# leavesnight/VIEO_SLAM

Hardware: AMD Instinct MI355X
Metric: frontend+localBA frames/sec on EuRoC MH05 stereo-VIO; ATE vs ref (higher is better)
Workload: dtype u8 (extract/match) + f64 (pose optimisation)

## Files before the change

vieo_slam_amd/csrc/matching.hip:

```cpp
#include <climits>

#include "orb_internal.h"
#include "wave_ops.h"

namespace vieo {

static const int TH_HIGH = 100, TH_LOW = 50;

__device__ __forceinline__ int hamming32(const uint4 a0, const uint4 a1, const uint8_t* b) {
  const uint4 b0 = ((const uint4*)b)[0], b1 = ((const uint4*)b)[1];
  return __popc(a0.x ^ b0.x) + __popc(a0.y ^ b0.y) + __popc(a0.z ^ b0.z) + __popc(a0.w ^ b0.w) +
         __popc(a1.x ^ b1.x) + __popc(a1.y ^ b1.y) + __popc(a1.z ^ b1.z) + __popc(a1.w ^ b1.w);
}

__device__ __forceinline__ bool lex_less(int d0, int i0, int d1, int i1) {
  return d0 < d1 || (d0 == d1 && i0 < i1);
}

struct Knn2Job {
  const uint8_t* q;
  const uint8_t* t;
  int nq, nt;
  int out_off;
};

struct Knn2Src {
  const Knn2Job* jobs;
  const uint8_t* desc;
  const int32_t* counts;
  int cap, n_cams, n_pairs;
  signed char pi[6], pj[6];
};

__global__ void __launch_bounds__(256)
k_knn2(Knn2Src S, int32_t* __restrict__ idx, int32_t* __restrict__ dist) {
  __shared__ uint4 s_t[256 * 2];
  __shared__ unsigned s_m[3][64][2];
  Knn2Job J;
  if (S.jobs)
    J = S.jobs[blockIdx.y];
  else {
    const int f = blockIdx.z, p = blockIdx.y, ci = S.pi[p], cj = S.pj[p];
    const int32_t* c = S.counts + (size_t)f * S.n_cams * 2;
    const int ni = c[2 * ci], mi = c[2 * ci + 1], nj = c[2 * cj], mj = c[2 * cj + 1];
    const bool skip = mi >= ni || mj >= nj;
    J.q = S.desc + (((size_t)f * S.n_cams + ci) * S.cap + mi) * 32;
    J.t = S.desc + (((size_t)f * S.n_cams + cj) * S.cap + mj) * 32;
    J.nq = skip ? 0 : min(ni, S.cap) - mi, J.nt = skip ? 0 : min(nj, S.cap) - mj;
    J.out_off = ((int)f * S.n_pairs + p) * S.cap;
  }
  const int lane = threadIdx.x & 63, wave = __builtin_amdgcn_readfirstlane((int)(threadIdx.x >> 6));
  const int q0 = blockIdx.x * 64;
  if (q0 >= J.nq) return;
  const int qi = q0 + lane;
  uint4 a0 = {0, 0, 0, 0}, a1 = a0;
  if (qi < J.nq) a0 = ((const uint4*)(J.q + (size_t)qi * 32))[0], a1 = ((const uint4*)(J.q + (size_t)qi * 32))[1];
  unsigned k0 = 0xFFFFFFFFu, k1 = 0xFFFFFFFFu;
  const uint4* T = (const uint4*)J.t;
  for (int t0 = 0; t0 < J.nt; t0 += 256) {
    __syncthreads();
    const int rows = min(256, J.nt - t0);
    for (int e = threadIdx.x; e < rows * 2; e += 256) s_t[e] = T[(size_t)t0 * 2 + e];
    __syncthreads();
    const int r1 = min(rows, wave * 64 + 64);
    for (int r = wave * 64; r < r1; r++) {
      const uint4 b0 = s_t[2 * r], b1 = s_t[2 * r + 1];
      const unsigned d = __popc(a0.x ^ b0.x) + __popc(a0.y ^ b0.y) + __popc(a0.z ^ b0.z) + __popc(a0.w ^ b0.w) +
                         __popc(a1.x ^ b1.x) + __popc(a1.y ^ b1.y) + __popc(a1.z ^ b1.z) + __popc(a1.w ^ b1.w);
      const unsigned key = (d << 16) | (unsigned)(t0 + r);
      k1 = min(max(key, k0), k1);
      k0 = min(k0, key);
    }
  }
  if (wave > 0) s_m[wave - 1][lane][0] = k0, s_m[wave - 1][lane][1] = k1;
  __syncthreads();
  if (wave == 0 && qi < J.nq) {
#pragma unroll
    for (int w = 0; w < 3; w++) {
      const unsigned b0 = s_m[w][lane][0], b1 = s_m[w][lane][1];
      const unsigned lo = min(k0, b0), hi = max(k0, b0);
      k1 = min(hi, min(k1, b1));
      k0 = lo;
    }
    int32_t* oi = idx + ((size_t)J.out_off + qi) * 2;
    int32_t* od = dist + ((size_t)J.out_off + qi) * 2;
    oi[0] = k0 == 0xFFFFFFFFu ? -1 : (int)(k0 & 0xFFFF), od[0] = k0 == 0xFFFFFFFFu ? INT_MAX : (int)(k0 >> 16);
    oi[1] = k1 == 0xFFFFFFFFu ? -1 : (int)(k1 & 0xFFFF), od[1] = k1 == 0xFFFFFFFFu ? INT_MAX : (int)(k1 >> 16);
  }
}

typedef int knn_v16i __attribute__((ext_vector_type(16)));
typedef int knn_v4i __attribute__((ext_vector_type(4)));

__device__ __forceinline__ unsigned knn_spread4(unsigned nib) { return (nib * 0x00204081u) & 0x01010101u; }
__device__ __forceinline__ knn_v4i knn_spread16(unsigned h) {
  knn_v4i r;
  r[0] = (int)knn_spread4(h & 15u), r[1] = (int)knn_spread4((h >> 4) & 15u);
  r[2] = (int)knn_spread4((h >> 8) & 15u), r[3] = (int)knn_spread4((h >> 12) & 15u);
  return r;
}

#ifndef VIEO_KNN2_TILE_ROWS
#define VIEO_KNN2_TILE_ROWS 32
#endif
__global__ void __launch_bounds__(256)
k_knn2_mfma(Knn2Src S, int32_t* __restrict__ idx, int32_t* __restrict__ dist) {
  constexpr int TR = VIEO_KNN2_TILE_ROWS, NSUB = TR / 32, CH = TR * 16;
  __shared__ knn_v4i s_a[2][CH];
  __shared__ __attribute__((aligned(16))) unsigned s_L[2][TR];
  Knn2Job J;
  if (S.jobs)
    J = S.jobs[blockIdx.y];
  else {
    const int f = blockIdx.z, p = blockIdx.y, ci = S.pi[p], cj = S.pj[p];
    const int32_t* c = S.counts + (size_t)f * S.n_cams * 2;
    const int ni = c[2 * ci], mi = c[2 * ci + 1], nj = c[2 * cj], mj = c[2 * cj + 1];
    const bool skip = mi >= ni || mj >= nj;
    J.q = S.desc + (((size_t)f * S.n_cams + ci) * S.cap + mi) * 32;
    J.t = S.desc + (((size_t)f * S.n_cams + cj) * S.cap + mj) * 32;
    J.nq = skip ? 0 : min(ni, S.cap) - mi, J.nt = skip ? 0 : min(nj, S.cap) - mj;
    J.out_off = ((int)f * S.n_pairs + p) * S.cap;
  }
  if ((int)blockIdx.x * 256 >= J.nq) return;
  const int tid = threadIdx.x, lane = tid & 63, wave = tid >> 6;
  const int j = lane & 31, g = lane >> 5;
  const int q0 = blockIdx.x * 256 + wave * 64;
  knn_v4i B[2][8];
  unsigned pb[2];
#pragma unroll
  for (int s = 0; s < 2; s++) {
    const int qi = q0 + 32 * s + j;
    uint4 h = {0, 0, 0, 0};
    if (qi < J.nq) h = ((const uint4*)(J.q + (size_t)qi * 32))[g];
    const unsigned half = __popc(h.x) + __popc(h.y) + __popc(h.z) + __popc(h.w);
    pb[s] = half + (unsigned)__shfl_xor((int)half, 32);
    const unsigned w[4] = {h.x, h.y, h.z, h.w};
#pragma unroll
    for (int m = 0; m < 8; m++) B[s][m] = knn_spread16((w[m >> 1] >> (16 * (m & 1))) & 0xFFFFu);
  }
  unsigned k0[2] = {0xFFFFFFFFu, 0xFFFFFFFFu}, k1[2] = {0xFFFFFFFFu, 0xFFFFFFFFu};
  const int n_tiles = (J.nt + TR - 1) / TR;
  constexpr int NU = CH / 256;
  unsigned h16[NU];
  uint4 ra = {0, 0, 0, 0}, rb = ra;
  auto fetch = [&](int T) {
#pragma unroll
    for (int u = 0; u < NU; u++) {
      const int cc = tid + 256 * u, sub = cc >> 9, m = (cc >> 6) & 7, gg = (cc >> 5) & 1, row = T * TR + sub * 32 + (cc & 31);
      h16[u] = row < J.nt ? (unsigned)*(const unsigned short*)(J.t + (size_t)row * 32 + 16 * gg + 2 * m) : 0u;
    }
    if (tid < TR) {
      const int row = T * TR + tid;
      ra = rb = make_uint4(0, 0, 0, 0);
      if (row < J.nt) ra = ((const uint4*)(J.t + (size_t)row * 32))[0], rb = ((const uint4*)(J.t + (size_t)row * 32))[1];
    }
  };
  auto stage = [&](int T, int b) {
#pragma unroll
    for (int u = 0; u < NU; u++) s_a[b][tid + 256 * u] = knn_spread16(h16[u]);
    if (tid < TR) {
      const int row = T * TR + tid;
      const unsigned pa = __popc(ra.x) + __popc(ra.y) + __popc(ra.z) + __popc(ra.w) + __popc(rb.x) + __popc(rb.y) + __popc(rb.z) + __popc(rb.w);
      s_L[b][tid] = row < J.nt ? ((pa + 512u) << 16) | (unsigned)row : 0xFFFFFFFFu;
    }
  };
  fetch(0);
  stage(0, 0);
  __syncthreads();
  for (int T = 0; T < n_tiles; T++) {
    const int b = T & 1;
    if (T + 1 < n_tiles) fetch(T + 1);
#pragma unroll
    for (int sub = 0; sub < NSUB; sub++) {
      knn_v16i acc0 = {0, 0, 0, 0, 0, 0, 0, 0, 0, 0, 0, 0, 0, 0, 0, 0}, acc1 = acc0;
#pragma unroll
      for (int m = 0; m < 8; m++) {
        const knn_v4i a = s_a[b][((sub * 8 + m) * 2 + g) * 32 + j];
        acc0 = __builtin_amdgcn_mfma_i32_32x32x32_i8(a, B[0][m], acc0, 0, 0, 0);
        acc1 = __builtin_amdgcn_mfma_i32_32x32x32_i8(a, B[1][m], acc1, 0, 0, 0);
      }
#pragma unroll
      for (int q4 = 0; q4 < 4; q4++) {
        const uint4 Lw = *(const uint4*)&s_L[b][sub * 32 + 8 * q4 + 4 * g];
        const unsigned L[4] = {Lw.x, Lw.y, Lw.z, Lw.w};
#pragma unroll
        for (int e = 0; e < 4; e++) {
          const unsigned ka = L[e] - ((unsigned)acc0[4 * q4 + e] << 17), kb = L[e] - ((unsigned)acc1[4 * q4 + e] << 17);
          k1[0] = min(max(ka, k0[0]), k1[0]), k0[0] = min(k0[0], ka);
          k1[1] = min(max(kb, k0[1]), k1[1]), k0[1] = min(k0[1], kb);
        }
      }
    }
    if (T + 1 < n_tiles) stage(T + 1, b ^ 1);
    __syncthreads();
  }
#pragma unroll
  for (int s = 0; s < 2; s++) {
    const unsigned o0 = (unsigned)__shfl_xor((int)k0[s], 32), o1 = (unsigned)__shfl_xor((int)k1[s], 32);
    const unsigned lo = min(k0[s], o0), hi = max(k0[s], o0);
    const unsigned second = min(hi, min(k1[s], o1));
    const int qi = q0 + 32 * s + j;
    if (g == 0 && qi < J.nq) {
      int32_t* oi = idx + ((size_t)J.out_off + qi) * 2;
      int32_t* od = dist + ((size_t)J.out_off + qi) * 2;
      oi[0] = lo == 0xFFFFFFFFu ? -1 : (int)(lo & 0xFFFF), od[0] = lo == 0xFFFFFFFFu ? INT_MAX : (int)(lo >> 16) - 512 + (int)pb[s];
      oi[1] = second == 0xFFFFFFFFu ? -1 : (int)(second & 0xFFFF);
      od[1] = second == 0xFFFFFFFFu ? INT_MAX : (int)(second >> 16) - 512 + (int)pb[s];
    }
  }
}

static bool knn2_mfma() {
  static const bool on = [] {
    const char* e = getenv("VIEO_KNN2_MFMA");
    return !e || atoi(e) != 0;
  }();
  return on;
}
static void knn2_launch(const Knn2Src& S, int max_nq, int ny, int nz, int32_t* d_idx, int32_t* d_dist, hipStream_t st) {
  if (knn2_mfma())
    hipLaunchKernelGGL(k_knn2_mfma, dim3((max_nq + 255) / 256, ny, nz), dim3(256), 0, st, S, d_idx, d_dist);
  else
    hipLaunchKernelGGL(k_knn2, dim3((max_nq + 63) / 64, ny, nz), dim3(256), 0, st, S, d_idx, d_dist);
}

int knn2_rig_launch(const uint8_t* d_desc, const int32_t* d_counts, int cap, int n_cams, int n_frames, int32_t* d_idx,
                    int32_t* d_dist, hipStream_t st) {
  Knn2Src S;
  memset(&S, 0, sizeof(S));
  S.desc = d_desc, S.counts = d_counts, S.cap = cap, S.n_cams = n_cams;
  int p = 0;
  for (int i = 0; i < n_cams - 1; i++)
    for (int j = i + 1; j < n_cams; j++, p++) S.pi[p] = (signed char)i, S.pj[p] = (signed char)j;
  S.n_pairs = p;
  if (p == 0 || n_frames <= 0) return VIEO_OK;
  knn2_launch(S, cap, p, n_frames, d_idx, d_dist, st);
  VIEO_HIP_CHECK(hipGetLastError());
  return VIEO_OK;
}

struct StereoArgs {
  OrbParams P;
  ImgSet IL, IR;
  int l_first, l_step, r_first, r_step;
  const vieo_keypoint *kpL, *kpR;
  const uint8_t *descL, *descR;
  const int *cntL, *cntR;
  int capL, capR;
  float baseline, bf;
  float* uright;
  float* depth;
  int* sad;
  int* row_start;
  int2* row_list;
  int H, list_cap;
};

__device__ __forceinline__ int wave_sum_i(int v) { return wave_sum_i32(v); }

template <int NT>
__global__ void __launch_bounds__(NT) k_stereo_rows(StereoArgs A) {
  extern __shared__ int s_rows[];
  __shared__ int s_part[16];
  const int f = blockIdx.x, tid = threadIdx.x, H = A.H;
  int* cnt = s_rows;
  int* cur = s_rows + H + 1;
  const int imR = A.r_first + f * A.r_step;
  const int Nr = min(A.cntR[2 * imR], A.capR);
  const vieo_keypoint* KR = A.kpR + (size_t)imR * A.capR;
  for (int y = tid; y <= H; y += NT) cnt[y] = 0;
  __syncthreads();
  for (int j = tid; j < Nr; j += NT) {
    const float y = KR[j].y, r = 2.0f * A.P.lv[KR[j].octave].scale;
    const int maxr = min((int)ceilf(y + r), H - 1), minr = max((int)floorf(y - r), 0);
    for (int yi = minr; yi <= maxr; yi++) atomicAdd(&cnt[yi], 1);
  }
  __syncthreads();
  const int per = (H + NT - 1) / NT, y0 = min(H, tid * per), y1 = min(H, y0 + per);
  int sum = 0;
  for (int y = y0; y < y1; y++) sum += cnt[y];
  int inc = sum;
  for (int o = 1; o < 64; o <<= 1) {
    const int t = __shfl_up(inc, o);
    if ((tid & 63) >= o) inc += t;
  }
  if ((tid & 63) == 63) s_part[tid >> 6] = inc;
  __syncthreads();
  int acc = inc - sum;
  for (int w = 0; w < (tid >> 6); w++) acc += s_part[w];
  int* rs = A.row_start + (size_t)f * (H + 1);
  for (int y = y0; y < y1; y++) {
    const int v = cnt[y];
    rs[y] = acc, cur[y] = acc;
    acc += v;
  }
  if (tid == NT - 1) rs[H] = acc;
  __syncthreads();
  int2* list = A.row_list + (size_t)f * A.list_cap;
  for (int j = tid; j < Nr; j += NT) {
    const vieo_keypoint kj = KR[j];
    const float y = kj.y, r = 2.0f * A.P.lv[kj.octave].scale;
    const int maxr = min((int)ceilf(y + r), H - 1), minr = max((int)floorf(y - r), 0);
    for (int yi = minr; yi <= maxr; yi++) {
      const int pos = atomicAdd(&cur[yi], 1);
      if (pos < A.list_cap) list[pos] = make_int2(j | (kj.octave << 20), __float_as_int(kj.x));
    }
  }
}

__device__ __forceinline__ unsigned row_min_u32(unsigned v) {
  v = min(v, (unsigned)VIEO_DPP(v, v, VIEO_DPP_QUAD_XOR1, 0xF));
  v = min(v, (unsigned)VIEO_DPP(v, v, VIEO_DPP_QUAD_XOR2, 0xF));
  v = min(v, (unsigned)VIEO_DPP(v, v, VIEO_DPP_ROW_HALF_MIRROR, 0xF));
  v = min(v, (unsigned)VIEO_DPP(v, v, VIEO_DPP_ROW_MIRROR, 0xF));
  return v;
}
__device__ __forceinline__ int row_sum_i32(int v) {
  v += VIEO_DPP(0, v, VIEO_DPP_QUAD_XOR1, 0xF);
  v += VIEO_DPP(0, v, VIEO_DPP_QUAD_XOR2, 0xF);
  v += VIEO_DPP(0, v, VIEO_DPP_ROW_HALF_MIRROR, 0xF);
  v += VIEO_DPP(0, v, VIEO_DPP_ROW_MIRROR, 0xF);
  return v;
}

__global__ void __launch_bounds__(256) k_stereo_rect(StereoArgs A) {
  const int f = blockIdx.y, lane = threadIdx.x & 63, g = lane >> 4, gl = lane & 15;
  const int wave = __builtin_amdgcn_readfirstlane((int)(threadIdx.x >> 6));
  const int iL = (blockIdx.x * 4 + wave) * 4 + g;
  const int imL = A.l_first + f * A.l_step, imR = A.r_first + f * A.r_step;
  const int N = min(A.cntL[2 * imL], A.capL);
  bool alive = iL < N;
  const int iLc = alive ? iL : 0;
  float* o_ur = A.uright + (size_t)f * A.capL + iLc;
  float* o_dp = A.depth + (size_t)f * A.capL + iLc;
  int* o_sad = A.sad + (size_t)f * A.capL + iLc;
  if (alive && gl == 0) *o_ur = -1.0f, *o_dp = -1.0f, *o_sad = -1;
  if (!__any(alive)) return;
  const vieo_keypoint kL = A.kpL[(size_t)imL * A.capL + iLc];
  const int levelL = kL.octave;
  const float vL = kL.y, uL = kL.x;
  const int rowL = (int)vL;
  const float minD = 0.f, maxD = A.bf / A.baseline;
  const float minU = uL - maxD, maxU = uL - minD;
  alive = alive && !(maxU < 0) && rowL >= 0 && rowL < A.H;
  const int rowc = min(max(rowL, 0), A.H - 1);
  const uint8_t* dL = A.descL + ((size_t)imL * A.capL + iLc) * 32;
  const uint4 a0 = ((const uint4*)dL)[0], a1 = ((const uint4*)dL)[1];
  const uint8_t* DR = A.descR + (size_t)imR * A.capR * 32;
  int bestDist = TH_HIGH, bestIdx = INT_MAX;
  float bestX = 0.f;
  const int* rs = A.row_start + (size_t)f * (A.H + 1);
  const int2* list = A.row_list + (size_t)f * A.list_cap;
  const int c0 = rs[rowc], c1 = alive ? min(rs[rowc + 1], A.list_cap) : c0;
  for (int cb = c0; __any(cb < c1); cb += 32) {
    int2 e[2];
    bool in[2];
#pragma unroll
    for (int u = 0; u < 2; u++) {
      const int c = cb + gl + 16 * u;
      in[u] = c < c1;
      e[u] = in[u] ? list[c] : make_int2(0, 0);
    }
    int dd[2];
#pragma unroll
    for (int u = 0; u < 2; u++) {
      const int j = e[u].x & 0xFFFFF, octR = e[u].x >> 20;
      const float xR = __int_as_float(e[u].y);
      in[u] = in[u] && !(octR < levelL - 1 || octR > levelL + 1) && (xR >= minU && xR <= maxU);
      dd[u] = in[u] ? hamming32(a0, a1, DR + (size_t)j * 32) : TH_HIGH;
    }
#pragma unroll
    for (int u = 0; u < 2; u++) {
      const int j = e[u].x & 0xFFFFF;
      if (in[u] && dd[u] < TH_HIGH && lex_less(dd[u], j, bestDist, bestIdx))
        bestDist = dd[u], bestIdx = j, bestX = __int_as_float(e[u].y);
    }
  }
  const int myIdx = bestIdx;
  {
    const unsigned m = row_min_u32(bestIdx == INT_MAX ? 0xFFFFFFFFu : ((unsigned)bestDist << 20) | (unsigned)bestIdx);
    bestIdx = m == 0xFFFFFFFFu ? INT_MAX : (int)(m & 0xFFFFF);
    bestDist = m == 0xFFFFFFFFu ? INT_MAX : (int)(m >> 20);
  }
  alive = alive && bestIdx != INT_MAX && bestDist < (TH_HIGH + TH_LOW) / 2;
  const unsigned long long own = __ballot(alive && myIdx == bestIdx);
  const unsigned own_g = (unsigned)((own >> (16 * g)) & 0xFFFFull);
  const int src_lane = g * 16 + (own_g ? __builtin_ffs((int)own_g) - 1 : 0);
  const float uR0 = __int_as_float(__builtin_amdgcn_ds_bpermute(src_lane * 4, __float_as_int(bestX)));
  const float sF = 1.0f / A.P.lv[levelL].scale;
  const float scaleduL = roundf(kL.x * sF), scaledvL = roundf(kL.y * sF);
  const float scaleduR0 = roundf(uR0 * sF);
  const int w = 5, L = 5;
  const float iniu = scaleduR0 + L - w, endu = scaleduR0 + L + w + 1;
  const int lvw = A.P.lv[levelL].w, lvh = A.P.lv[levelL].h;
  alive = alive && !(iniu < 0 || endu >= (float)lvw);
  if (!__any(alive)) return;
  int pitchL, pitchR;
  const uint8_t* PL = plane_ptr(A.P, A.IL, imL, levelL, &pitchL);
  const uint8_t* PR = plane_ptr(A.P, A.IR, imR, levelL, &pitchR);
  const int r0 = (int)(scaledvL - w), cL0 = (int)(scaleduL - w), cR0 = (int)(scaleduR0 - w);
  auto clampy = [&](int yy) { return min(max(yy, 0), lvh - 1); };
  auto clampx = [&](int xx) { return min(max(xx, 0), lvw - 1); };
  const int cvL = alive ? (int)PL[(size_t)(r0 + w) * pitchL + cL0 + w] : 0;
  int py[8], px[8], il[8];
#pragma unroll
  for (int k = 0; k < 8; k++) {
    const int p = gl + 16 * k;
    py[k] = p / 11, px[k] = p - py[k] * 11;
    il[k] = (alive && p < 121) ? (int)PL[(size_t)clampy(r0 + py[k]) * pitchL + clampx(cL0 + px[k])] - cvL : 0;
  }
  __shared__ uint8_t s_strip[16][11 * 21 + 25];
  uint8_t* strip = s_strip[wave * 4 + g];
  {
    unsigned v[15];
#pragma unroll
    for (int k = 0; k < 15; k++) {
      const int p = gl + 16 * k, row = p / 21, col = p - row * 21;
      v[k] = (alive && p < 231) ? PR[(size_t)clampy(r0 + row) * pitchR + clampx(cR0 - L + col)] : 0;
    }
#pragma unroll
    for (int k = 0; k < 15; k++)
      if (gl + 16 * k < 231) strip[gl + 16 * k] = (uint8_t)v[k];
  }
  __builtin_amdgcn_fence(__ATOMIC_RELEASE, "wavefront");
  __builtin_amdgcn_wave_barrier();
  __builtin_amdgcn_fence(__ATOMIC_ACQUIRE, "wavefront");
  int bestS = INT_MAX, bestInc = 0, sads[11];
#pragma unroll
  for (int inc = -L; inc <= L; inc++) {
    const int cvR = strip[w * 21 + inc + L + w];
    int acc = 0;
#pragma unroll
    for (int k = 0; k < 8; k++) {
      if (gl + 16 * k < 121) {
        const int ir = (int)strip[py[k] * 21 + inc + L + px[k]] - cvR;
        acc += abs(il[k] - ir);
      }
    }
    acc = row_sum_i32(acc);
    sads[inc + L] = acc;
    if (acc < bestS) bestS = acc, bestInc = inc;
  }
  if (!alive || bestInc == -L || bestInc == L) return;
  float dist1 = 0, dist2 = 0, dist3 = 0;
#pragma unroll
  for (int k = 1; k < 10; k++)
    if (k == bestInc + L) dist1 = (float)sads[k - 1], dist2 = (float)sads[k], dist3 = (float)sads[k + 1];
  const float deltaR = (dist1 - dist3) / (2.0f * (dist1 + dist3 - 2.0f * dist2));
  if (deltaR < -1 || deltaR > 1) return;
  float bestuR = A.P.lv[levelL].scale * ((float)scaleduR0 + (float)bestInc + deltaR);
  float disparity = uL - bestuR;
  if (disparity >= minD && disparity < maxD) {
    if (disparity <= 0) {
      disparity = 0.01f;
      bestuR = (float)((double)uL - 0.01);
    }
    if (gl == 0) {
      *o_dp = A.bf / disparity;
      *o_ur = bestuR;
      *o_sad = bestS;
    }
  }
}

__global__ void __launch_bounds__(256) k_stereo_median(StereoArgs A) {
  __shared__ int s_part[2][4];
  const int f = blockIdx.x, tid = threadIdx.x, lane = tid & 63, wave = tid >> 6;
  const int imL = A.l_first + f * A.l_step;
  const int N = min(A.cntL[2 * imL], A.capL);
  int* sad = A.sad + (size_t)f * A.capL;
  constexpr int kR = 8;
  int v[kR];
#pragma unroll
  for (int r = 0; r < kR; r++) {
    const int i = tid + 256 * r;
    v[r] = i < N ? sad[i] : -1;
  }
  const bool spill = N > 256 * kR;
  auto block_count = [&](int bound, int slot) -> int {
    int c = 0;
#pragma unroll
    for (int r = 0; r < kR; r++) c += (v[r] >= 0 && v[r] <= bound);
    if (spill)
      for (int i = tid + 256 * kR; i < N; i += 256) {
        const int s = sad[i];
        c += (s >= 0 && s <= bound);
      }
    c = wave_sum_i32(c);
    if (lane == 0) s_part[slot][wave] = c;
    __syncthreads();
    return s_part[slot][0] + s_part[slot][1] + s_part[slot][2] + s_part[slot][3];
  };
  const int n = block_count((1 << 30), 0);
  if (n == 0) return;
  const int k = n / 2;
  int lo = 0, hi = (1 << 17) - 1;
  int slot = 1;
  while (lo < hi) {
    const int mid = (lo + hi) >> 1;
    const int cnt = block_count(mid, slot);
    slot ^= 1;
    if (cnt >= k + 1)
      hi = mid;
    else
      lo = mid + 1;
  }
  const float median = (float)lo;
  const float thDist = 1.5f * 1.4f * median;
  for (int i = tid; i < N; i += 256) {
    const int s = sad[i];
    if (s >= 0 && !((float)s < thDist)) {
      A.uright[(size_t)f * A.capL + i] = -1;
      A.depth[(size_t)f * A.capL + i] = -1;
    }
  }
}

static thread_local DevBuf g_row_start, g_row_list;

static int launch_stereo(StereoArgs A, int n_frames, hipStream_t st) {
  int rc;
  float smax = 1.f;
  for (int l = 0; l < A.P.nlevels; l++) smax = std::max(smax, A.P.lv[l].scale);
  A.H = A.P.lv[0].h;
  if (A.capR >= (1 << 20)) {
    set_error("ComputeStereoMatches: more than 2^20 keys per image");
    return VIEO_E_CAPACITY;
  }
  A.list_cap = A.capR * (2 * (int)ceilf(2.0f * smax) + 3);
  if ((rc = g_row_start.ensure((size_t)n_frames * (A.H + 1) * 4)) != VIEO_OK) return rc;
  if ((rc = g_row_list.ensure((size_t)n_frames * A.list_cap * 8)) != VIEO_OK) return rc;
  A.row_start = g_row_start.as<int>(), A.row_list = g_row_list.as<int2>();
  if (n_frames <= 16)
    hipLaunchKernelGGL(k_stereo_rows<1024>, dim3(n_frames), dim3(1024), (size_t)(2 * A.H + 1) * 4, st, A);
  else
    hipLaunchKernelGGL(k_stereo_rows<256>, dim3(n_frames), dim3(256), (size_t)(2 * A.H + 1) * 4, st, A);
  hipLaunchKernelGGL(k_stereo_rect, dim3((A.capL + 15) / 16, n_frames), dim3(256), 0, st, A);
  hipLaunchKernelGGL(k_stereo_median, dim3(n_frames), dim3(256), 0, st, A);
  VIEO_HIP_CHECK(hipGetLastError());
  return VIEO_OK;
}

static int same_geometry(const vieo_orb* a, const vieo_orb* b) {
  if (a->w != b->w || a->h != b->h || a->nlevels != b->nlevels || a->w == 0) return 0;
  for (int l = 0; l < a->nlevels; l++)
    if (a->P.lv[l].w != b->P.lv[l].w || a->P.lv[l].h != b->P.lv[l].h ||
        a->P.lv[l].scale != b->P.lv[l].scale)
      return 0;
  return 1;
}

struct MatchScratch {
  DevBuf kpL, kpR, dL, dR, cL, cR, ur, dp, sad, jobs, idx, dist;
};
static thread_local MatchScratch g_ms;

}

using namespace vieo;

extern "C" {

int vieo_stereo_match_rectified_batch_device(vieo_orb* e, int n_frames,
                                             const vieo_keypoint* d_keypoints,
                                             const uint8_t* d_descriptors, const int32_t* d_counts,
                                             int capacity, float baseline, float bf,
                                             float* d_uright, float* d_depth) {
  if (!e || n_frames <= 0 || 2 * n_frames > e->last_B || !d_keypoints || !d_descriptors ||
      !d_counts || !d_uright || !d_depth || !(baseline > 0) || !(bf > 0)) {
    set_error("vieo_stereo_match_rectified_batch_device: invalid arguments (the extractor's last "
              "batch must hold 2*n_frames images, left/right interleaved)");
    return VIEO_E_INVALID;
  }
  int rc;
  static thread_local DevBuf sad;
  if ((rc = sad.ensure((size_t)n_frames * capacity * 4)) != VIEO_OK) return rc;
  StereoArgs A;
  A.P = e->P;
  A.IL = A.IR = e->last_imgs;
  A.l_first = 0, A.l_step = 2, A.r_first = 1, A.r_step = 2;
  A.kpL = A.kpR = d_keypoints;
  A.descL = A.descR = d_descriptors;
  A.cntL = A.cntR = d_counts;
  A.capL = A.capR = capacity;
  A.baseline = baseline;
  A.bf = bf;
  A.uright = d_uright;
  A.depth = d_depth;
  A.sad = sad.as<int>();
  return launch_stereo(A, n_frames, e->stream);
}

int vieo_stereo_match_rectified(vieo_orb* left, vieo_orb* right, const vieo_keypoint* h_kpL,
                                const uint8_t* h_descL, int nL, const vieo_keypoint* h_kpR,
                                const uint8_t* h_descR, int nR, float baseline, float bf,
                                float* h_uright, float* h_depth) {
  if (!left || !right || nL < 0 || nR < 0 || !h_uright || !h_depth || !(baseline > 0) || !(bf > 0))
    return VIEO_E_INVALID;
  if (left->last_B < 1 || right->last_B < 1 || !same_geometry(left, right)) {
    set_error("vieo_stereo_match_rectified: both extractors must have processed equally sized "
              "images (their pyramids are read in place)");
    return VIEO_E_INVALID;
  }
  if (nL == 0) return VIEO_OK;
  int rc;
  MatchScratch& S = g_ms;
  const int capL = nL, capR = std::max(nR, 1);
#define ENS(b, n) \
  if ((rc = (b).ensure(n)) != VIEO_OK) return rc
  ENS(S.kpL, (size_t)capL * sizeof(vieo_keypoint));
  ENS(S.kpR, (size_t)capR * sizeof(vieo_keypoint));
  ENS(S.dL, (size_t)capL * 32);
  ENS(S.dR, (size_t)capR * 32);
  ENS(S.cL, 8);
  ENS(S.cR, 8);
  ENS(S.ur, (size_t)capL * 4);
  ENS(S.dp, (size_t)capL * 4);
  ENS(S.sad, (size_t)capL * 4);
#undef ENS
  hipStream_t st = left->stream;
  VIEO_HIP_CHECK(hipStreamSynchronize(right->stream));
  const int cl[2] = {nL, 0}, cr[2] = {nR, 0};
  VIEO_HIP_CHECK(hipMemcpyAsync(S.kpL.p, h_kpL, (size_t)nL * sizeof(vieo_keypoint), hipMemcpyHostToDevice, st));
  VIEO_HIP_CHECK(hipMemcpyAsync(S.dL.p, h_descL, (size_t)nL * 32, hipMemcpyHostToDevice, st));
  if (nR > 0) {
    VIEO_HIP_CHECK(hipMemcpyAsync(S.kpR.p, h_kpR, (size_t)nR * sizeof(vieo_keypoint), hipMemcpyHostToDevice, st));
    VIEO_HIP_CHECK(hipMemcpyAsync(S.dR.p, h_descR, (size_t)nR * 32, hipMemcpyHostToDevice, st));
  }
  VIEO_HIP_CHECK(hipMemcpyAsync(S.cL.p, cl, 8, hipMemcpyHostToDevice, st));
  VIEO_HIP_CHECK(hipMemcpyAsync(S.cR.p, cr, 8, hipMemcpyHostToDevice, st));
  StereoArgs A;
  A.P = left->P;
  A.IL = left->last_imgs;
  A.IR = right->last_imgs;
  A.l_first = 0, A.l_step = 0, A.r_first = 0, A.r_step = 0;
  A.kpL = S.kpL.as<vieo_keypoint>(), A.kpR = S.kpR.as<vieo_keypoint>();
  A.descL = S.dL.as<uint8_t>(), A.descR = S.dR.as<uint8_t>();
  A.cntL = S.cL.as<int>(), A.cntR = S.cR.as<int>();
  A.capL = capL, A.capR = capR;
  A.baseline = baseline, A.bf = bf;
  A.uright = S.ur.as<float>(), A.depth = S.dp.as<float>(), A.sad = S.sad.as<int>();
  if ((rc = launch_stereo(A, 1, st)) != VIEO_OK) return rc;
  VIEO_HIP_CHECK(hipMemcpyAsync(h_uright, S.ur.p, (size_t)nL * 4, hipMemcpyDeviceToHost, st));
  VIEO_HIP_CHECK(hipMemcpyAsync(h_depth, S.dp.p, (size_t)nL * 4, hipMemcpyDeviceToHost, st));
  VIEO_HIP_CHECK(hipStreamSynchronize(st));
  return VIEO_OK;
}

int vieo_stereo_match_rectified_resident(vieo_orb* left, vieo_orb* right, float baseline, float bf, float* h_uright,
                                         float* h_depth) {
  if (!left || !right || !h_uright || !h_depth || !(baseline > 0) || !(bf > 0)) return VIEO_E_INVALID;
  if (left->res_n < 0 || right->res_n < 0) {
    set_error("vieo_stereo_match_rectified_resident: a handle holds no frame (vieo_orb_extract first)");
    return VIEO_E_INVALID;
  }
  if (left->last_B < 1 || right->last_B < 1 || !same_geometry(left, right)) {
    set_error("vieo_stereo_match_rectified_resident: both extractors must have processed equally sized images");
    return VIEO_E_INVALID;
  }
  const int nL = left->res_n, capL = vieo_orb_max_keypoints(left), capR = vieo_orb_max_keypoints(right);
  int rc;
  if ((rc = left->d_uright.ensure((size_t)capL * 4)) != VIEO_OK || (rc = left->d_depth.ensure((size_t)capL * 4)) != VIEO_OK ||
      (rc = left->d_sad.ensure((size_t)capL * 4)) != VIEO_OK || (rc = left->h_io.ensure((size_t)capL * 8)) != VIEO_OK)
    return rc;
  left->uright_epoch = left->epoch;
  left->uright_host.clear();
  if (nL == 0) return VIEO_OK;
  hipStream_t st = left->stream;
  VIEO_HIP_CHECK(hipStreamSynchronize(right->stream));
  StereoArgs A;
  A.P = left->P;
  A.IL = left->last_imgs;
  A.IR = right->last_imgs;
  A.l_first = 0, A.l_step = 0, A.r_first = 0, A.r_step = 0;
  A.kpL = left->d_kp.as<vieo_keypoint>(), A.kpR = right->d_kp.as<vieo_keypoint>();
  A.descL = left->d_desc.as<uint8_t>(), A.descR = right->d_desc.as<uint8_t>();
  A.cntL = left->d_counts.as<int>(), A.cntR = right->d_counts.as<int>();
  A.capL = capL, A.capR = capR;
  A.baseline = baseline, A.bf = bf;
  A.uright = left->d_uright.as<float>(), A.depth = left->d_depth.as<float>(), A.sad = left->d_sad.as<int>();
  if ((rc = launch_stereo(A, 1, st)) != VIEO_OK) return rc;
  float* H = (float*)left->h_io.p;
  VIEO_HIP_CHECK(hipMemcpyAsync(H, left->d_uright.p, (size_t)nL * 4, hipMemcpyDeviceToHost, st));
  VIEO_HIP_CHECK(hipMemcpyAsync(H + capL, left->d_depth.p, (size_t)nL * 4, hipMemcpyDeviceToHost, st));
  VIEO_HIP_CHECK(hipStreamSynchronize(st));
  memcpy(h_uright, H, (size_t)nL * 4);
  memcpy(h_depth, H + capL, (size_t)nL * 4);
  left->uright_host.assign(H, H + nL);
  return VIEO_OK;
}

int vieo_hamming_knn2_batch_device(const uint8_t* d_descriptors, const int32_t* h_counts,
                                   int capacity, const int32_t* h_pairs, int n_pairs,
                                   int32_t* d_idx, int32_t* d_dist, void* stream) {
  if (!d_descriptors || !h_counts || !h_pairs || n_pairs <= 0 || !d_idx || !d_dist || capacity <= 0 || capacity > 65535)
    return VIEO_E_INVALID;
  int rc = require_device();
  if (rc != VIEO_OK) return rc;
  std::vector<Knn2Job> jobs(n_pairs);
  int max_nq = 0;
  for (int p = 0; p < n_pairs; p++) {
    const int qi = h_pairs[2 * p], ti = h_pairs[2 * p + 1];
    const int qm = h_counts[2 * qi + 1], tm = h_counts[2 * ti + 1];
    jobs[p].q = d_descriptors + ((size_t)qi * capacity + qm) * 32;
    jobs[p].t = d_descriptors + ((size_t)ti * capacity + tm) * 32;
    jobs[p].nq = std::max(h_counts[2 * qi] - qm, 0);
    jobs[p].nt = std::max(h_counts[2 * ti] - tm, 0);
    jobs[p].out_off = p * capacity;
    max_nq = std::max(max_nq, jobs[p].nq);
  }
  MatchScratch& S = g_ms;
  if ((rc = S.jobs.ensure(jobs.size() * sizeof(Knn2Job))) != VIEO_OK) return rc;
  hipStream_t st = (hipStream_t)stream;
  VIEO_HIP_CHECK(hipMemcpyAsync(S.jobs.p, jobs.data(), jobs.size() * sizeof(Knn2Job),
                                hipMemcpyHostToDevice, st));
  VIEO_HIP_CHECK(hipStreamSynchronize(st));
  if (max_nq > 0) {
    Knn2Src K;
    memset(&K, 0, sizeof(K));
    K.jobs = S.jobs.as<Knn2Job>();
    knn2_launch(K, max_nq, n_pairs, 1, d_idx, d_dist, st);
  }
  VIEO_HIP_CHECK(hipGetLastError());
  return VIEO_OK;
}

int vieo_hamming_knn2_rig_batch_device(const uint8_t* d_descriptors, const int32_t* d_counts, int capacity, int n_cams,
                                       int n_frames, int32_t* d_idx, int32_t* d_dist, void* stream) {
  if (!d_descriptors || !d_counts || capacity <= 0 || capacity > 65535 || n_cams < 2 || n_cams > 4 || n_frames <= 0 || !d_idx ||
      !d_dist)
    return VIEO_E_INVALID;
  int rc = require_device();
  if (rc != VIEO_OK) return rc;
  return knn2_rig_launch(d_descriptors, d_counts, capacity, n_cams, n_frames, d_idx, d_dist, (hipStream_t)stream);
}

int vieo_hamming_knn2(const uint8_t* h_query, int nq, const uint8_t* h_train, int nt,
                      int32_t* h_idx, int32_t* h_dist) {
  if (nq < 0 || nt < 0 || (nq > 0 && (!h_query || !h_idx || !h_dist))) return VIEO_E_INVALID;
  int rc = require_device();
  if (rc != VIEO_OK) return rc;
  if (nq == 0) return VIEO_OK;
  if (nt > 65535) {
    set_error("vieo_hamming_knn2: %d train rows, at most 65535", nt);
    return VIEO_E_CAPACITY;
  }
  MatchScratch& S = g_ms;
#define ENS(b, n) \
  if ((rc = (b).ensure(n)) != VIEO_OK) return rc
  ENS(S.dL, (size_t)nq * 32);
  ENS(S.dR, (size_t)std::max(nt, 1) * 32);
  ENS(S.idx, (size_t)nq * 8);
  ENS(S.dist, (size_t)nq * 8);
  ENS(S.jobs, sizeof(Knn2Job));
#undef ENS
  VIEO_HIP_CHECK(hipMemcpy(S.dL.p, h_query, (size_t)nq * 32, hipMemcpyHostToDevice));
  if (nt > 0) VIEO_HIP_CHECK(hipMemcpy(S.dR.p, h_train, (size_t)nt * 32, hipMemcpyHostToDevice));
  Knn2Job j;
  j.q = S.dL.as<uint8_t>(), j.t = S.dR.as<uint8_t>(), j.nq = nq, j.nt = nt, j.out_off = 0;
  VIEO_HIP_CHECK(hipMemcpy(S.jobs.p, &j, sizeof(j), hipMemcpyHostToDevice));
  Knn2Src K;
  memset(&K, 0, sizeof(K));
  K.jobs = S.jobs.as<Knn2Job>();
  knn2_launch(K, nq, 1, 1, S.idx.as<int32_t>(), S.dist.as<int32_t>(), 0);
  VIEO_HIP_CHECK(hipGetLastError());
  VIEO_HIP_CHECK(hipMemcpy(h_idx, S.idx.p, (size_t)nq * 8, hipMemcpyDeviceToHost));
  VIEO_HIP_CHECK(hipMemcpy(h_dist, S.dist.p, (size_t)nq * 8, hipMemcpyDeviceToHost));
  return VIEO_OK;
}

}
```

Before: 60440.

## Add packed-SAD fast path for stereo refinement and widen candidate list unroll

Adds a fast path for the stereo SAD window search. Each lane loads one 11-pixel row of the left and right patches as aligned dwords, shifts them with alignbyte, and computes all 11 disparity offsets using packed u16 sad instructions. This avoids the shared-memory strip and the per-pixel byte loads. Interior windows use this path, while border or misaligned cases fall back to the old strip-based code. The per-lane SAD results are then reduced with a DPP min/max to find the best offset and its neighbours. The change also caches the level table in LDS, unrolls the candidate-list loop three times, and hoists the descriptor loads, at the cost of more register pressure and a new __syncthreads.

```diff
diff --git a/vieo_slam_amd/csrc/matching.hip b/vieo_slam_amd/csrc/matching.hip
--- a/vieo_slam_amd/csrc/matching.hip
+++ b/vieo_slam_amd/csrc/matching.hip
@@ -309,10 +309,17 @@
 }
 
 __device__ __forceinline__ unsigned row_min_u32(unsigned v) {
-  v = min(v, (unsigned)VIEO_DPP(v, v, VIEO_DPP_QUAD_XOR1, 0xF));
-  v = min(v, (unsigned)VIEO_DPP(v, v, VIEO_DPP_QUAD_XOR2, 0xF));
-  v = min(v, (unsigned)VIEO_DPP(v, v, VIEO_DPP_ROW_HALF_MIRROR, 0xF));
-  v = min(v, (unsigned)VIEO_DPP(v, v, VIEO_DPP_ROW_MIRROR, 0xF));
+  v = min(v, (unsigned)VIEO_DPP(0xFFFFFFFFu, v, VIEO_DPP_QUAD_XOR1, 0xF));
+  v = min(v, (unsigned)VIEO_DPP(0xFFFFFFFFu, v, VIEO_DPP_QUAD_XOR2, 0xF));
+  v = min(v, (unsigned)VIEO_DPP(0xFFFFFFFFu, v, VIEO_DPP_ROW_HALF_MIRROR, 0xF));
+  v = min(v, (unsigned)VIEO_DPP(0xFFFFFFFFu, v, VIEO_DPP_ROW_MIRROR, 0xF));
+  return v;
+}
+__device__ __forceinline__ unsigned row_max_u32(unsigned v) {
+  v = max(v, (unsigned)VIEO_DPP(0, v, VIEO_DPP_QUAD_XOR1, 0xF));
+  v = max(v, (unsigned)VIEO_DPP(0, v, VIEO_DPP_QUAD_XOR2, 0xF));
+  v = max(v, (unsigned)VIEO_DPP(0, v, VIEO_DPP_ROW_HALF_MIRROR, 0xF));
+  v = max(v, (unsigned)VIEO_DPP(0, v, VIEO_DPP_ROW_MIRROR, 0xF));
   return v;
 }
 __device__ __forceinline__ int row_sum_i32(int v) {
@@ -323,20 +330,50 @@
   return v;
 }
 
+#ifndef VIEO_STEREO_LIST_U
+#define VIEO_STEREO_LIST_U 3
+#endif
+
+struct alignas(16) StereoLevel {
+  float scale, inv_scale;
+  int w, h, off, pitch, pad0, pad1;
+};
+struct __attribute__((packed, aligned(4))) StereoDw4 { unsigned v[4]; };
+struct __attribute__((packed, aligned(4))) StereoDw2 { unsigned v[2]; };
+
+__device__ __forceinline__ unsigned pk_add_u16(unsigned a, unsigned b) {
+  typedef unsigned short u16x2 __attribute__((ext_vector_type(2)));
+  return __builtin_bit_cast(unsigned, (u16x2)(__builtin_bit_cast(u16x2, a) + __builtin_bit_cast(u16x2, b)));
+}
+__device__ __forceinline__ unsigned byte_pair16(const unsigned* R, int c) {
+  const unsigned lo = c & 3, hi = lo == 3 ? 4u : lo + 1u;
+  return __builtin_amdgcn_perm(R[(c + 1) >> 2], R[c >> 2], lo | 0x0c00u | (hi << 16) | 0x0c000000u);
+}
+__device__ __forceinline__ unsigned byte_splat16(const unsigned* R, int c) {
+  const unsigned b = c & 3;
+  return __builtin_amdgcn_perm(R[c >> 2], R[c >> 2], b | 0x0c00u | (b << 16) | 0x0c000000u);
+}
+
 __global__ void __launch_bounds__(256) k_stereo_rect(StereoArgs A) {
+  __shared__ StereoLevel s_lv[kMaxLevels];
   const int f = blockIdx.y, lane = threadIdx.x & 63, g = lane >> 4, gl = lane & 15;
   const int wave = __builtin_amdgcn_readfirstlane((int)(threadIdx.x >> 6));
   const int iL = (blockIdx.x * 4 + wave) * 4 + g;
   const int imL = A.l_first + f * A.l_step, imR = A.r_first + f * A.r_step;
+  const int iLc = min(iL, A.capL - 1);
+  const vieo_keypoint kL = A.kpL[(size_t)imL * A.capL + iLc];
+  const uint8_t* dL = A.descL + ((size_t)imL * A.capL + iLc) * 32;
+  const uint4 a0 = ((const uint4*)dL)[0], a1 = ((const uint4*)dL)[1];
+  if (threadIdx.x < kMaxLevels) {
+    const LevelDesc& d = A.P.lv[threadIdx.x];
+    s_lv[threadIdx.x] = StereoLevel{d.scale, 1.0f / d.scale, d.w, d.h, d.off, d.pitch, 0, 0};
+  }
+  __syncthreads();
   const int N = min(A.cntL[2 * imL], A.capL);
   bool alive = iL < N;
-  const int iLc = alive ? iL : 0;
-  float* o_ur = A.uright + (size_t)f * A.capL + iLc;
-  float* o_dp = A.depth + (size_t)f * A.capL + iLc;
-  int* o_sad = A.sad + (size_t)f * A.capL + iLc;
-  if (alive && gl == 0) *o_ur = -1.0f, *o_dp = -1.0f, *o_sad = -1;
+  const size_t o_base = (size_t)f * A.capL;
+  if (alive && gl == 0) A.uright[o_base + iL] = -1.0f, A.depth[o_base + iL] = -1.0f, A.sad[o_base + iL] = -1;
   if (!__any(alive)) return;
-  const vieo_keypoint kL = A.kpL[(size_t)imL * A.capL + iLc];
   const int levelL = kL.octave;
   const float vL = kL.y, uL = kL.x;
   const int rowL = (int)vL;
@@ -344,33 +381,32 @@
   const float minU = uL - maxD, maxU = uL - minD;
   alive = alive && !(maxU < 0) && rowL >= 0 && rowL < A.H;
   const int rowc = min(max(rowL, 0), A.H - 1);
-  const uint8_t* dL = A.descL + ((size_t)imL * A.capL + iLc) * 32;
-  const uint4 a0 = ((const uint4*)dL)[0], a1 = ((const uint4*)dL)[1];
   const uint8_t* DR = A.descR + (size_t)imR * A.capR * 32;
   int bestDist = TH_HIGH, bestIdx = INT_MAX;
   float bestX = 0.f;
   const int* rs = A.row_start + (size_t)f * (A.H + 1);
   const int2* list = A.row_list + (size_t)f * A.list_cap;
   const int c0 = rs[rowc], c1 = alive ? min(rs[rowc + 1], A.list_cap) : c0;
-  for (int cb = c0; __any(cb < c1); cb += 32) {
-    int2 e[2];
-    bool in[2];
-#pragma unroll
-    for (int u = 0; u < 2; u++) {
+  constexpr int U = VIEO_STEREO_LIST_U;
+  for (int cb = c0; __any(cb < c1); cb += 16 * U) {
+    int2 e[U];
+    bool in[U];
+#pragma unroll
+    for (int u = 0; u < U; u++) {
       const int c = cb + gl + 16 * u;
       in[u] = c < c1;
       e[u] = in[u] ? list[c] : make_int2(0, 0);
     }
-    int dd[2];
-#pragma unroll
-    for (int u = 0; u < 2; u++) {
+    int dd[U];
+#pragma unroll
+    for (int u = 0; u < U; u++) {
       const int j = e[u].x & 0xFFFFF, octR = e[u].x >> 20;
       const float xR = __int_as_float(e[u].y);
       in[u] = in[u] && !(octR < levelL - 1 || octR > levelL + 1) && (xR >= minU && xR <= maxU);
       dd[u] = in[u] ? hamming32(a0, a1, DR + (size_t)j * 32) : TH_HIGH;
     }
 #pragma unroll
-    for (int u = 0; u < 2; u++) {
+    for (int u = 0; u < U; u++) {
       const int j = e[u].x & 0xFFFFF;
       if (in[u] && dd[u] < TH_HIGH && lex_less(dd[u], j, bestDist, bestIdx))
         bestDist = dd[u], bestIdx = j, bestX = __int_as_float(e[u].y);
@@ -387,68 +423,137 @@
   const unsigned own_g = (unsigned)((own >> (16 * g)) & 0xFFFFull);
   const int src_lane = g * 16 + (own_g ? __builtin_ffs((int)own_g) - 1 : 0);
   const float uR0 = __int_as_float(__builtin_amdgcn_ds_bpermute(src_lane * 4, __float_as_int(bestX)));
-  const float sF = 1.0f / A.P.lv[levelL].scale;
+  const StereoLevel lv = s_lv[levelL & (kMaxLevels - 1)];
+  const float sF = lv.inv_scale;
   const float scaleduL = roundf(kL.x * sF), scaledvL = roundf(kL.y * sF);
   const float scaleduR0 = roundf(uR0 * sF);
   const int w = 5, L = 5;
   const float iniu = scaleduR0 + L - w, endu = scaleduR0 + L + w + 1;
-  const int lvw = A.P.lv[levelL].w, lvh = A.P.lv[levelL].h;
+  const int lvw = lv.w, lvh = lv.h;
   alive = alive && !(iniu < 0 || endu >= (float)lvw);
   if (!__any(alive)) return;
-  int pitchL, pitchR;
-  const uint8_t* PL = plane_ptr(A.P, A.IL, imL, levelL, &pitchL);
-  const uint8_t* PR = plane_ptr(A.P, A.IR, imR, levelL, &pitchR);
+  const int pitchL = levelL == 0 ? A.IL.stride0 : lv.pitch, pitchR = levelL == 0 ? A.IR.stride0 : lv.pitch;
+  const uint8_t* PL = levelL == 0 ? A.IL.img0 + (size_t)imL * A.IL.img_pitch : A.IL.pyr + (size_t)imL * A.IL.pyr_img + lv.off;
+  const uint8_t* PR = levelL == 0 ? A.IR.img0 + (size_t)imR * A.IR.img_pitch : A.IR.pyr + (size_t)imR * A.IR.pyr_img + lv.off;
   const int r0 = (int)(scaledvL - w), cL0 = (int)(scaleduL - w), cR0 = (int)(scaleduR0 - w);
-  auto clampy = [&](int yy) { return min(max(yy, 0), lvh - 1); };
-  auto clampx = [&](int xx) { return min(max(xx, 0), lvw - 1); };
-  const int cvL = alive ? (int)PL[(size_t)(r0 + w) * pitchL + cL0 + w] : 0;
-  int py[8], px[8], il[8];
-#pragma unroll
-  for (int k = 0; k < 8; k++) {
-    const int p = gl + 16 * k;
-    py[k] = p / 11, px[k] = p - py[k] * 11;
-    il[k] = (alive && p < 121) ? (int)PL[(size_t)clampy(r0 + py[k]) * pitchL + clampx(cL0 + px[k])] - cvL : 0;
-  }
-  __shared__ uint8_t s_strip[16][11 * 21 + 25];
-  uint8_t* strip = s_strip[wave * 4 + g];
-  {
-    unsigned v[15];
-#pragma unroll
-    for (int k = 0; k < 15; k++) {
-      const int p = gl + 16 * k, row = p / 21, col = p - row * 21;
-      v[k] = (alive && p < 231) ? PR[(size_t)clampy(r0 + row) * pitchR + clampx(cR0 - L + col)] : 0;
-    }
-#pragma unroll
-    for (int k = 0; k < 15; k++)
-      if (gl + 16 * k < 231) strip[gl + 16 * k] = (uint8_t)v[k];
-  }
-  __builtin_amdgcn_fence(__ATOMIC_RELEASE, "wavefront");
-  __builtin_amdgcn_wave_barrier();
-  __builtin_amdgcn_fence(__ATOMIC_ACQUIRE, "wavefront");
-  int bestS = INT_MAX, bestInc = 0, sads[11];
-#pragma unroll
-  for (int inc = -L; inc <= L; inc++) {
-    const int cvR = strip[w * 21 + inc + L + w];
-    int acc = 0;
+  const int cS0 = cR0 - L;
+  const bool fast = alive && r0 >= 0 && r0 + 2 * w < lvh && cL0 >= 0 && cL0 + 2 * w < lvw && cS0 >= 0 && cS0 + 2 * (w + L) < lvw &&
+                    ((((uintptr_t)PL | (uintptr_t)PR) | (uintptr_t)(unsigned)(pitchL | pitchR)) & 3) == 0 &&
+                    (cL0 & ~3) + 16 <= pitchL && (cS0 & ~3) + 24 <= pitchR;
+  const bool slow = alive && !fast;
+  unsigned sad_own = 0;
+  if (__any(fast)) {
+    const int row = r0 + min(gl, 2 * w);
+    const uint8_t* pl = PL + (size_t)row * pitchL + (cL0 & ~3);
+    const uint8_t* pr = PR + (size_t)row * pitchR + (cS0 & ~3);
+    const uint8_t* pc = PR + (size_t)(r0 + w) * pitchR + (cS0 & ~3) + 4;
+    StereoDw4 l4 = {{0, 0, 0, 0}}, r4 = l4, c4 = l4;
+    StereoDw2 r2 = {{0, 0}};
+    unsigned cvL = 0;
+    if (fast) {
+      l4 = *(const StereoDw4*)pl;
+      r4 = *(const StereoDw4*)pr;
+      r2 = *(const StereoDw2*)(pr + 16);
+      c4 = *(const StereoDw4*)pc;
+      cvL = PL[(size_t)(r0 + w) * pitchL + cL0 + w];
+    }
+    const unsigned sL = cL0 & 3, sR = cS0 & 3;
+    const unsigned rr[7] = {r4.v[0], r4.v[1], r4.v[2], r4.v[3], r2.v[0], r2.v[1], 0u};
+    unsigned Lb[3], Rb[6], Cb[3];
+#pragma unroll
+    for (int k = 0; k < 3; k++) Lb[k] = __builtin_amdgcn_alignbyte(l4.v[k + 1], l4.v[k], sL);
+#pragma unroll
+    for (int k = 0; k < 6; k++) Rb[k] = __builtin_amdgcn_alignbyte(rr[k + 1], rr[k], sR);
+#pragma unroll
+    for (int k = 0; k < 3; k++) Cb[k] = __builtin_amdgcn_alignbyte(c4.v[k + 1], c4.v[k], sR);
+    const unsigned cvL2 = cvL * 0x10001u;
+    unsigned ILp[5], IRe[10], IRo[10], IRs[11];
+#pragma unroll
+    for (int k = 0; k < 5; k++) ILp[k] = byte_pair16(Lb, 2 * k);
+    const unsigned il10 = (Lb[2] >> 16) & 0xFFu;
+#pragma unroll
+    for (int k = 0; k < 10; k++) {
+      IRe[k] = pk_add_u16(byte_pair16(Rb, 2 * k), cvL2);
+      IRo[k] = pk_add_u16(byte_pair16(Rb, 2 * k + 1), cvL2);
+    }
+#pragma unroll
+    for (int c = 10; c <= 20; c++) IRs[c - 10] = c == 20 ? IRo[9] >> 16 : ((c & 1) ? IRo[(c - 1) / 2] : IRe[c / 2]) & 0xFFFFu;
+    const bool counts = fast && gl <= 2 * w;
+    unsigned P[6];
+#pragma unroll
+    for (int i = 0; i <= 2 * L; i++) {
+      const unsigned cvR2 = byte_splat16(Cb, i + 1);
+      unsigned a = 0;
+#pragma unroll
+      for (int k = 0; k < 5; k++)
+        a = __builtin_amdgcn_sad_u16(pk_add_u16(ILp[k], cvR2), (i & 1) ? IRo[(i + 2 * k - 1) / 2] : IRe[(i + 2 * k) / 2], a);
+      a = __builtin_amdgcn_sad_u16(il10 + (cvR2 & 0xFFFFu), IRs[i], a);
+      if (i & 1)
+        P[i >> 1] |= a << 16;
+      else
+        P[i >> 1] = a;
+    }
+    unsigned pk = 0;
+#pragma unroll
+    for (int k = 0; k < 6; k++) {
+      const unsigned s = (unsigned)row_sum_i32((int)(counts ? P[k] : 0u));
+      pk = (gl >> 1) == k ? s : pk;
+    }
+    if (fast) sad_own = (gl & 1) ? pk >> 16 : pk & 0xFFFFu;
+  }
+  if (__any(slow)) {
+    const bool alive = slow;
+    auto clampy = [&](int yy) { return min(max(yy, 0), lvh - 1); };
+    auto clampx = [&](int xx) { return min(max(xx, 0), lvw - 1); };
+    const int cvL = alive ? (int)PL[(size_t)(r0 + w) * pitchL + cL0 + w] : 0;
+    int py[8], px[8], il[8];
 #pragma unroll
     for (int k = 0; k < 8; k++) {
-      if (gl + 16 * k < 121) {
-        const int ir = (int)strip[py[k] * 21 + inc + L + px[k]] - cvR;
-        acc += abs(il[k] - ir);
+      const int p = gl + 16 * k;
+      py[k] = p / 11, px[k] = p - py[k] * 11;
+      il[k] = (alive && p < 121) ? (int)PL[(size_t)clampy(r0 + py[k]) * pitchL + clampx(cL0 + px[k])] - cvL : 0;
+    }
+    __shared__ uint8_t s_strip[16][11 * 21 + 25];
+    uint8_t* strip = s_strip[wave * 4 + g];
+    {
+      unsigned v[15];
+#pragma unroll
+      for (int k = 0; k < 15; k++) {
+        const int p = gl + 16 * k, row = p / 21, col = p - row * 21;
+        v[k] = (alive && p < 231) ? PR[(size_t)clampy(r0 + row) * pitchR + clampx(cR0 - L + col)] : 0;
       }
-    }
-    acc = row_sum_i32(acc);
-    sads[inc + L] = acc;
-    if (acc < bestS) bestS = acc, bestInc = inc;
-  }
+#pragma unroll
+      for (int k = 0; k < 15; k++)
+        if (gl + 16 * k < 231) strip[gl + 16 * k] = (uint8_t)v[k];
+    }
+    __builtin_amdgcn_fence(__ATOMIC_RELEASE, "wavefront");
+    __builtin_amdgcn_wave_barrier();
+    __builtin_amdgcn_fence(__ATOMIC_ACQUIRE, "wavefront");
+    int mine = 0;
+#pragma unroll
+    for (int inc = -L; inc <= L; inc++) {
+      const int cvR = strip[w * 21 + inc + L + w];
+      int acc = 0;
+#pragma unroll
+      for (int k = 0; k < 8; k++) {
+        if (gl + 16 * k < 121) {
+          const int ir = (int)strip[py[k] * 21 + inc + L + px[k]] - cvR;
+          acc += abs(il[k] - ir);
+        }
+      }
+      acc = row_sum_i32(acc);
+      mine = gl == inc + L ? acc : mine;
+    }
+    if (alive) sad_own = (unsigned)mine;
+  }
+  const unsigned mkey = row_min_u32(gl <= 2 * L ? (sad_own << 4) | (unsigned)gl : 0xFFFFFFFFu);
+  const int bestS = (int)(mkey >> 4), bi = (int)(mkey & 15u), bestInc = bi - L;
+  const unsigned s1 = row_max_u32(gl == bi - 1 ? sad_own : 0u), s3 = row_max_u32(gl == bi + 1 ? sad_own : 0u);
   if (!alive || bestInc == -L || bestInc == L) return;
-  float dist1 = 0, dist2 = 0, dist3 = 0;
-#pragma unroll
-  for (int k = 1; k < 10; k++)
-    if (k == bestInc + L) dist1 = (float)sads[k - 1], dist2 = (float)sads[k], dist3 = (float)sads[k + 1];
+  const float dist1 = (float)s1, dist2 = (float)bestS, dist3 = (float)s3;
   const float deltaR = (dist1 - dist3) / (2.0f * (dist1 + dist3 - 2.0f * dist2));
   if (deltaR < -1 || deltaR > 1) return;
-  float bestuR = A.P.lv[levelL].scale * ((float)scaleduR0 + (float)bestInc + deltaR);
+  float bestuR = lv.scale * ((float)scaleduR0 + (float)bestInc + deltaR);
   float disparity = uL - bestuR;
   if (disparity >= minD && disparity < maxD) {
     if (disparity <= 0) {
@@ -456,9 +561,9 @@
       bestuR = (float)((double)uL - 0.01);
     }
     if (gl == 0) {
-      *o_dp = A.bf / disparity;
-      *o_ur = bestuR;
-      *o_sad = bestS;
+      A.depth[o_base + iL] = A.bf / disparity;
+      A.uright[o_base + iL] = bestuR;
+      A.sad[o_base + iL] = bestS;
     }
   }
 }
```

New measurement: 60360. Within noise of the previous version (-0.1%).
